# KyleHuang9/YOLO-LP

Measured on AMD Instinct MI355X. Metric: images/sec (640×640) end-to-end detect+NMS, yololps, 1/2/4/8 MI355X, higher is better.
Workload: dtype f16; 1 GPU; yololps 640x640 bs=32/GPU f16, synthetic frames resident in HBM, seeded random-init weights (sigma 0.25), conf 0.40 iou 0.45 max_det 1000; global_batch=32, parallelism=dp1: images sharded, all-gather of detections

## Files before the change

include/lp_hip.h:

```cpp
#ifndef LP_HIP_H
#define LP_HIP_H

#include <stddef.h>
#include <stdint.h>

#ifdef __cplusplus
extern "C" {
#endif

typedef enum { LP_OK = 0, LP_ERR_ARG = -1, LP_ERR_STATE = -2, LP_ERR_HIP = -3, LP_ERR_UNSUPPORTED = -4 } lp_status;
typedef enum { LP_F16 = 0, LP_BF16 = 1, LP_F32 = 2 } lp_dtype;
typedef enum { LP_ACT_NONE = 0, LP_ACT_RELU = 1, LP_ACT_SILU = 2 } lp_act;

#define LP_PRED_COLS 290
#define LP_DET_COLS 28
#define LP_MAX_SRC 4

typedef struct lp_engine lp_engine;

const char* lp_version(void);
const char* lp_last_error(void);

int lp_engine_create(lp_engine** out, int act_dtype );
void lp_engine_destroy(lp_engine* e);
// ... 201 lines not shown
    uint16_t taps[LP_REDACT_MAX_RADIUS + 1];
    uint16_t taps_c[LP_REDACT_MAX_RADIUS + 1];
} lp_redact_gauss_params;
size_t lp_redact_gauss_workspace_bytes(const lp_redact_desc* desc, int n_frames, const lp_redact_gauss_params* p);
int lp_redact_gauss_batch(const lp_redact_desc* desc, int n_frames, const float* det, const int32_t* count, int max_det,
                          const lp_redact_gauss_params* p, int32_t* status ,
                          void* workspace, size_t workspace_bytes, void* stream);

#define LP_LOOKBACK_MAX_DEPTH 32
size_t lp_lookback_state_bytes(int n_streams, int max_tracks, int depth, int rows);
int lp_lookback_update(void* state, int n_streams, int max_tracks, int depth, int max_back, int back_cap,
                       const float* det_hold, const int32_t* count_hold, const int32_t* tid, const int32_t* slot,
                       int B, int max_det, int hold_rows,
                       const int* stream_of , const unsigned char* flush ,
                       float* rel_det, int32_t* rel_count, int32_t* rel_frame,
                       float* tail_det, int32_t* tail_count, int32_t* tail_frame, void* stream);

#define LP_WATCH_MAX_ENTRIES (1 << 24)
#define LP_WATCH_MAX_COST 32768
#define LP_WATCH_BLOCK_ENTRIES 2048
#define LP_WATCH_QUERY_BLOCK 16
size_t lp_watch_workspace_bytes(int n_streams, int max_ended);
int lp_watch_match(const unsigned char* entries, int n_entries, const unsigned char* confuse ,
                   const int32_t* ended_i, const float* ended_f, const int32_t* ended_count, int n_streams, int max_ended,
                   int max_mismatch, int max_cost, int32_t* match_i, void* workspace, size_t workspace_bytes, void* stream);

#define LP_MERGE_MAX_TILES 64
#define LP_TILE_GATE_TILE_WORDS 8
typedef struct lp_tile_gate_desc {
    const unsigned char* p0;
    int pitch0;
    int h0, w0;
    int format;
    unsigned short* blocks;
} lp_tile_gate_desc;
int lp_tile_gate_luma_batch(const lp_tile_gate_desc* desc, int n_frames, void* stream);
int lp_tile_gate_update(const lp_tile_gate_desc* desc, int n_frames, const int* stream_of , int n_streams,
                        const int32_t* tiles, const int* n_tiles , int max_tiles,
                        unsigned short* ref, long long ref_elems, int32_t* age, int thres16, int min_cells, int refresh,
                        unsigned char* flag, int32_t* ncell, void* stream);

enum { LP_EVAL_TRUE = 0, LP_EVAL_PRED = 1, LP_EVAL_PRED_BINS = 2, LP_EVAL_COR = 12, LP_EVAL_CLS = 22, LP_EVAL_RIGHT = 32,
       LP_EVAL_UNBINNED = 42, LP_EVAL_NCOUNTS = 43 };
int lp_eval_counts(const float* det, const int32_t* det_count, int max_det, const float* tgt, const int32_t* tgt_count,
                   int max_t, int B, long long* counts, void* stream);

int lp_check_sigmoid_monotone(unsigned long long* dev_violations, void* stream);

int lp_check_iou_predicate(const float* dev_pairs, long long n, double iou_thres, unsigned char* dev_out, void* stream);

int lp_debug_poison_lds(void* stream);

int lp_plan_stem_tile(int fused, int Ho, int Wo, int choice, int* TH, int* TW, int* hpitch);
int lp_plan_block_tile(int variant, int Ho, int Wo, int B, int nct, int choice, int* TH, int* TW, int* hpitch);

#ifdef __cplusplus
}
#endif
#endif
```

yolo-lp_amd/csrc/lp_conv.hip:

```cpp
#include "lp_internal.h"

#include <cstdlib>

namespace lp {

int conv_launch_f16(int cfg, int mode, int ksize, int stride, int nbuf, const ConvArgs& a, hipStream_t st);
int conv_launch_bf16(int cfg, int mode, int ksize, int stride, int nbuf, const ConvArgs& a, hipStream_t st);
int conv_launch_f32(int cfg, int mode, int ksize, int stride, int nbuf, const ConvArgs& a, hipStream_t st);

int conv_stream_launch_f16(int wc, const ConvArgs& a, int cb_pack, int lds, hipStream_t st);
int conv_stream_launch_bf16(int wc, const ConvArgs& a, int cb_pack, int lds, hipStream_t st);
int conv_stream_launch_f32(int wc, const ConvArgs& a, int cb_pack, int lds, hipStream_t st);

int conv_pipe_launch_f16(int pcfg, const ConvArgs& a, int ncu, hipStream_t st);
int conv_pipe_launch_bf16(int pcfg, const ConvArgs& a, int ncu, hipStream_t st);

int head_rows_launch_f16(const ConvArgs& a, int cb_pack, hipStream_t st);
int head_rows_launch_bf16(const ConvArgs& a, int cb_pack, hipStream_t st);
int head_rows_launch_f32(const ConvArgs& a, int cb_pack, hipStream_t st);
int head_box_det_launch_f16(const ConvArgs& a, int cb_pack, hipStream_t st);
int head_box_det_launch_bf16(const ConvArgs& a, int cb_pack, hipStream_t st);
int head_box_det_launch_f32(const ConvArgs& a, int cb_pack, hipStream_t st);

ConvShape conv_shape(int dtype, int cfg, int ksize, int stride) {
// ... 226 lines not shown
    const ConvShape s = conv_pipe_shape(pcfg);
    if (pipe_is_16v(pcfg) && (nct * s.CB > 512 || nchunks > 32)) return false;
    return s.CB == cb_pack && nct * s.CB <= 1024 && nchunks <= 64;
}

static int g_ncu[16] = {0};
int device_cus() {
    int dev = 0;
    if (hipGetDevice(&dev) != hipSuccess || dev < 0 || dev >= 16) return 256;
    if (!g_ncu[dev]) {
        int n = 0;
        if (hipDeviceGetAttribute(&n, hipDeviceAttributeMultiprocessorCount, dev) != hipSuccess || n < 8) n = 256;
        g_ncu[dev] = n / 8 * 8;
        if (const char* cap = getenv("LP_PIPE_MAXWG")) { const int c = atoi(cap) / 8 * 8; if (c >= 8 && c < g_ncu[dev]) g_ncu[dev] = c; }
    }
    return g_ncu[dev];
}

bool stem_planar_tile(int Ho, int Wo, int choice, int* TH, int* TW) {
    struct Cand { long long tiles; int th, tw; };
    std::vector<Cand> cands;
    for (int tw = 4; tw <= 512 && tw < Wo + 4; tw += 4) {
        int th = 512 / tw;
        if (th > Ho) th = Ho;
        while (th >= 1 && ((th + 2) * 6 + 2) * (tw / 4 + 2) * 16 > 20 * 1024) --th;
        if (th < 1) continue;
        cands.push_back({(long long)ceil_div(Ho, th) * ceil_div(Wo, tw), th, tw});
    }
    std::sort(cands.begin(), cands.end(), [](const Cand& x, const Cand& y) { return x.tiles != y.tiles ? x.tiles < y.tiles : x.tw > y.tw; });
    if (choice < 0 || choice >= (int)cands.size()) return false;
    *TH = cands[choice].th;
    *TW = cands[choice].tw;
    return true;
}

bool stem2_fused_tile(int Ho, int Wo, int choice, int* TH, int* TW, int* hpitch) {
    struct Cand { long long cost; int th, tw; };
    std::vector<Cand> cands;
    for (int tw = 2; tw <= 128 && tw < Wo + 2; tw += 2)
        for (int th = 1; th <= 128 / tw && th <= Ho; ++th) {
            const int hp4 = tw / 2 + 2, rin = 2 * th + 3, hps = 2 * tw + 1;
            const int ntb = (th * tw + 31) / 32;
            if ((rin * 6 + 2) * hp4 * 16 > 21 * 1024 || (rin * 6 * hp4 + 63) / 64 > 24 || (2 * th + 1) * hps > 640 || ntb * 2 > 16) continue;
            cands.push_back({(long long)ceil_div(Ho, th) * ceil_div(Wo, tw) * (2 * th + 1) * hps, th, tw});
        }
    std::sort(cands.begin(), cands.end(), [](const Cand& x, const Cand& y) { return x.cost != y.cost ? x.cost < y.cost : x.tw > y.tw; });
    if (choice < 0 || choice >= (int)cands.size()) return false;
    *TH = cands[choice].th;
    *TW = cands[choice].tw;
    *hpitch = 2 * cands[choice].tw + 1;
    return true;
}

int conv_pipe_launch(int dtype, int pcfg, const ConvArgs& a, hipStream_t st) {
    if (pcfg == PIPE_P || pcfg == PIPE_FUSED2 || pcfg == PIPE_FUSED_PW || pcfg == PIPE_FUSED_BF) {
        switch (dtype) {
            case LP_F16: return conv_pipe_launch_f16(pcfg, a, device_cus(), st);
            case LP_BF16: return conv_pipe_launch_bf16(pcfg, a, device_cus(), st);
        }
        return fail(LP_ERR_UNSUPPORTED, "planar stem: 16-bit frames only");
    }
    const ConvShape s = conv_pipe_shape(pcfg);
    if (pipe_is_16s2(pcfg)) {
        const int hh2 = 2 * a.TH + 1, hw2 = 2 * a.TW + 1, nchunks = a.chunk_begin[a.nsrc];
        if (a.TH < 1 || a.TW < 1 || a.TH * a.TW > s.PB || a.hpitch != hw2 || hh2 * a.hpitch > s.HPMAX)
            return fail(LP_ERR_ARG, "conv3x3 s2p16: tile does not fit the kernel configuration");
        if (a.tiles_x * a.TW < a.Wo || a.tiles_y * a.TH < a.Ho) return fail(LP_ERR_ARG, "conv3x3 s2p16: tiles do not cover the output");
        if (a.nsrc < 1 || a.nsrc > LP_MAX_SRC || a.nct < 1 || a.nct * s.CB > 512 || nchunks < 1 || nchunks > 64 || a.nphase != 1 || a.out_scale != 1 ||
            a.H != 2 * a.Ho || a.W != 2 * a.Wo || a.out2)
            return fail(LP_ERR_ARG, "conv3x3 s2p16: not a 3x3 stride-2 layer this kernel runs");
        const int stride = a.out_pix_stride > a.res_cs ? a.out_pix_stride : a.res_cs;
        if (((long long)a.TH * a.Wo + a.TW) * stride + 2048 >= (1ll << 31)) return fail(LP_ERR_ARG, "conv3x3 s2p16: a tile's rows span more than 2^31 elements");
        switch (dtype) {
            case LP_F16: return conv_pipe_launch_f16(pcfg, a, device_cus(), st);
            case LP_BF16: return conv_pipe_launch_bf16(pcfg, a, device_cus(), st);
        }
        return fail(LP_ERR_UNSUPPORTED, "conv3x3 s2p16: 16-bit activations only");
    }
    const int hh = a.TH + 2, hw = a.TW + 2;
    if (pcfg < 0 || (pcfg >= PIPE_COUNT && !pipe_is_16(pcfg))) return fail(LP_ERR_ARG, "conv3x3 pipe: configuration");
    if (pipe_is_16(pcfg) && (a.chunk_begin[a.nsrc] < 4 || a.chunk_begin[a.nsrc] % 4 != 0)) return fail(LP_ERR_ARG, "conv3x3 pipe16: K-chunks not a multiple of four");
    if (a.TH < 1 || a.TW < 1 || a.TH * a.TW > s.PB || a.hpitch < hw || hh * a.hpitch > s.HPMAX)
        return fail(LP_ERR_ARG, "conv3x3 pipe: tile does not fit the kernel configuration");
    if (a.tiles_x * a.TW < a.Wo || a.tiles_y * a.TH < a.Ho) return fail(LP_ERR_ARG, "conv3x3 pipe: tiles do not cover the output");
    if (pipe_is_16v(pcfg) && (a.nct * s.CB > 512 || a.chunk_begin[a.nsrc] > 32)) return fail(LP_ERR_ARG, "conv3x3 pipe16v: layer exceeds the kernel's LDS tables");
    if (pipe_is_16v(pcfg)) {
        int stride = a.out_pix_stride > a.res_cs ? a.out_pix_stride : a.res_cs;
        if (a.out2 && a.out2_pix_stride > stride) stride = a.out2_pix_stride;
        if (((long long)a.TH * a.Wo + a.TW) * stride + 2048 >= (1ll << 31)) return fail(LP_ERR_ARG, "conv3x3 pipe16v: a tile's rows span more than 2^31 elements");
    }
    if (a.chunk_begin[a.nsrc] > 64) return fail(LP_ERR_ARG, "conv3x3 pipe: more K-chunks than the kernel's LDS chunk table holds");
    if (a.nsrc < 1 || a.nsrc > LP_MAX_SRC || a.nct < 1 || a.nct * s.CB > 1024 || a.nphase != 1 || a.out_scale != 1 || a.Ho != a.H || a.Wo != a.W)
        return fail(LP_ERR_ARG, "conv3x3 pipe: not a 3x3 stride-1 layer this kernel runs");
    switch (dtype) {
        case LP_F16: return conv_pipe_launch_f16(pcfg, a, device_cus(), st);
        case LP_BF16: return conv_pipe_launch_bf16(pcfg, a, device_cus(), st);
    }
    return fail(LP_ERR_UNSUPPORTED, "conv3x3 pipe: 16-bit activations only");
}

bool head_rows_fits(int dtype, int nchunks, int cb_pack, int out_c) {
    const long lds = (long)nchunks * 9 * 32 * 128 + 9 * 32 * 4 + 32 * 8 + 32 * 1168;
    return nchunks >= 1 && nchunks <= 3 && lds <= 160 * 1024 && (cb_pack == 32 || cb_pack == 64 || cb_pack == 128) && out_c == LP_PRED_COLS - 13;
}
bool head_det_fits(int dtype, int nchunks, int cb_pack, int out_c) {
    const long lds = (long)nchunks * 9 * 32 * 128 + 9 * 32 * 4 + 32 * 8 * 4 + 16 + 6 * 32 * 8 * 4 + 6 * 1168;
    return nchunks >= 1 && nchunks <= (dtype == LP_F32 ? 3 : 4) && lds <= 160 * 1024 && (cb_pack == 32 || cb_pack == 64 || cb_pack == 128) &&
           out_c == LP_PRED_COLS - 13;
}

bool head_box_det_fits(const ConvArgs& a, int cb_pack, int ksize, int stride) {
    const int nchunks = a.chunk_begin[a.nsrc];
    return ksize == 1 && stride == 1 && a.nsrc == 1 && nchunks >= 1 && nchunks <= 4 && a.reg_bins == 1 && a.out_c == 12 && a.nct == 1 &&
           cb_pack >= 32 && a.nphase == 1 && a.out_scale == 1 && a.Ho == a.H && a.Wo == a.W && a.src[0].cs % 8 == 0;
}
int head_box_det_launch(int dtype, const ConvArgs& a, int cb_pack, hipStream_t st) {
    if (!a.det_mode || !a.out || !a.zero || !head_box_det_fits(a, cb_pack, 1, 1)) return fail(LP_ERR_ARG, "head box: op does not fit");
    if (a.out_pix_stride % 4 != 0 || a.out_img_stride % 4 != 0 || ((uintptr_t)a.out & 15)) return fail(LP_ERR_ARG, "head box: candidate rows are not 16-byte aligned");
    switch (dtype) {
        case LP_F16: return head_box_det_launch_f16(a, cb_pack, st);
        case LP_BF16: return head_box_det_launch_bf16(a, cb_pack, st);
        case LP_F32: return head_box_det_launch_f32(a, cb_pack, st);
    }
    return fail(LP_ERR_ARG, "head box: dtype");
}

int head_rows_launch(int dtype, const ConvArgs& a, int cb_pack, hipStream_t st) {
    const int nchunks = a.chunk_begin[a.nsrc];
    if (!(a.det_mode ? head_det_fits(dtype, nchunks, cb_pack, a.out_c) : head_rows_fits(dtype, nchunks, cb_pack, a.out_c)))
        return fail(LP_ERR_ARG, "head rows: op does not fit");
    const int kc = 128 / (int)dtype_size(dtype);
    for (int i = 0; i < a.nsrc; ++i)
        if (a.src[i].cs % (kc / 4) != 0)
            return fail(LP_ERR_ARG, "head rows: source channels are not whole 32-byte K-steps");
    if (a.nphase != 1 || a.out_scale != 1 || a.Ho != a.H || a.Wo != a.W || !a.out) return fail(LP_ERR_ARG, "head rows: bad geometry");
    switch (dtype) {
        case LP_F16: return head_rows_launch_f16(a, cb_pack, st);
        case LP_BF16: return head_rows_launch_bf16(a, cb_pack, st);
        case LP_F32: return head_rows_launch_f32(a, cb_pack, st);
    }
    return fail(LP_ERR_ARG, "head rows: dtype");
}

}

extern "C" int lp_plan_block_tile(int variant, int Ho, int Wo, int B, int nct, int choice, int* TH, int* TW, int* hpitch) {
    const int pcfg = variant - LP_VARIANT_PIPE_D;
    if (!TH || !TW || Ho < 1 || Wo < 1 || B < 1 || nct < 1) return lp::fail(LP_ERR_ARG, "lp_plan_block_tile: bad arguments");
    if (!lp::pipe_is_16v(pcfg) && !lp::pipe_is_16s2(pcfg)) return lp::fail(LP_ERR_UNSUPPORTED, "lp_plan_block_tile: not a block-tiled variant");
    const lp::ConvShape s = lp::conv_pipe_shape(pcfg);
    const int stride = lp::pipe_is_16s2(pcfg) ? 2 : 1;
    lp::conv_pick_tile16v(s, Ho, Wo, B, nct, choice, TH, TW, stride);
    if (hpitch) *hpitch = (*TW - 1) * stride + 3;
    return LP_OK;
}

extern "C" int lp_plan_stem_tile(int fused, int Ho, int Wo, int choice, int* TH, int* TW, int* hpitch) {
    if (!TH || !TW || Ho < 1 || Wo < 1) return lp::fail(LP_ERR_ARG, "lp_plan_stem_tile: bad arguments");
    int hp = 0;
    const bool ok = fused ? lp::stem2_fused_tile(Ho, Wo, choice, TH, TW, &hp) : lp::stem_planar_tile(Ho, Wo, choice, TH, TW);
    if (hpitch) *hpitch = hp;
    return ok ? LP_OK : LP_ERR_UNSUPPORTED;
}
```

yolo-lp_amd/csrc/lp_engine.hip:

```cpp
#include "lp_internal.h"

#include <cmath>
#include <cstdlib>
#include <cstring>
#include <map>
#include <utility>
#include <vector>

namespace lp {

static thread_local std::string g_err;
void set_error(const std::string& msg) { g_err = msg; }
int fail(int code, const std::string& msg) {
    g_err = msg;
    return code;
}

enum OpKind { OP_INPUT = 0, OP_CONV = 1, OP_DECONV = 2, OP_POOL = 3, OP_HEAD_CLS = 4, OP_HEAD_BOX = 5 };

struct Tensor {
    int c, cs, sl;
    bool unused = false;
    size_t offset;
    int h, w;
// ... 761 lines not shown
    L.cb_pack = cb_pack;
    if (op.planar) {
        Launch& P = e->stem_planar;
        P = L;
        ConvArgs& pa = P.a;
        if (pa.W % 4 != 0 || !stem_planar_tile(pa.Ho, pa.Wo, op.planar - 1, &pa.TH, &pa.TW))
            return fail(LP_ERR_UNSUPPORTED, "planar stem: no tile for this frame size");
        pa.tw_magic = (unsigned)(((1u << 22) + pa.TW - 1) / pa.TW);
        pa.tiles_x = ceil_div(pa.Wo, pa.TW);
        pa.tiles_y = ceil_div(pa.Ho, pa.TH);
        pa.src[0].ptr = nullptr;
        P.pipe = PIPE_P + 1;
    }
    if (op.fused) {
        const Op& stem = e->ops[1];
        Launch& F = e->stem2_fused;
        F = L;
        ConvArgs& fa = F.a;
        if (!stem2_fused_tile(fa.Ho, fa.Wo, op.fused - 1, &fa.TH, &fa.TW, &fa.hpitch))
            return fail(LP_ERR_UNSUPPORTED, "fused stem: no tile for this frame size");
        fa.tw_magic = (unsigned)(((1u << 22) + fa.TW - 1) / fa.TW);
        fa.hp_magic = (unsigned)(((1u << 22) + fa.hpitch - 1) / fa.hpitch);
        fa.tiles_x = ceil_div(fa.Wo, fa.TW);
        fa.tiles_y = ceil_div(fa.Ho, fa.TH);
        fa.src[0].ptr = nullptr;
        fa.fz_w1 = e->dev_w + stem.w_off;
        fa.fz_b1 = (const float*)(e->dev_w + stem.b_off);
        fa.fz_act1 = stem.act;
        fa.fz_c1 = e->tensors[stem.dst].cs;
        F.pipe = PIPE_FUSED2 + 1;
    }
    if (op.fused_bf) {
        const Op& up = e->ops[op.bf_up];
        const Op& c1 = e->ops[op.bf_cv1];
        Launch& F = e->bf_fused[(int)idx];
        F = L;
        ConvArgs& fa = F.a;
        fa.src[0].ptr = tptr(up.src[0]); fa.src[0].cs = e->tensors[up.src[0]].cs;
        fa.src[1].ptr = tptr(c1.src[0]); fa.src[1].cs = e->tensors[c1.src[0]].cs;
        fa.fz_w1 = e->dev_w + c1.w_off;
        fa.fz_b1 = (const float*)(e->dev_w + c1.b_off);
        fa.fz_act1 = c1.act;
        fa.bf_wd = e->dev_w + up.w_off;
        fa.bf_bd = (const float*)(e->dev_w + up.b_off);
        fa.bf_wd_phase_stride = up.w_phase_stride;
        F.pipe = PIPE_FUSED_BF + 1;
    }
    if (op.fused_pw) {
        const Op& pw = e->ops[idx - 1];
        Launch& F = e->pw_fused[(int)idx];
        F = L;
        ConvArgs& fa = F.a;
        int hp = 0;
        if (!stem2_fused_tile(fa.Ho, fa.Wo, op.fused_pw - 1, &fa.TH, &fa.TW, &hp))
            return fail(LP_ERR_UNSUPPORTED, "fused 1x1 + 3x3 s2: no tile for this map size");
        fa.hpitch = hp;
        fa.tw_magic = (unsigned)(((1u << 22) + fa.TW - 1) / fa.TW);
        fa.hp_magic = (unsigned)(((1u << 22) + fa.hpitch - 1) / fa.hpitch);
        fa.tiles_x = ceil_div(fa.Wo, fa.TW);
        fa.tiles_y = ceil_div(fa.Ho, fa.TH);
        fa.src[0].ptr = tptr(pw.src[0]);
        fa.src[0].cs = e->tensors[pw.src[0]].cs;
        fa.fz_w1 = e->dev_w + pw.w_off;
        fa.fz_b1 = (const float*)(e->dev_w + pw.b_off);
        fa.fz_act1 = pw.act;
        fa.fz_c1 = e->tensors[pw.dst].cs;
        F.pipe = PIPE_FUSED_PW + 1;
    }
    return LP_OK;
}

static bool stem_planar_possible(const lp_engine* e) {
    return e->dtype != LP_F32 && e->ops.size() > 1 && e->ops[0].kind == OP_INPUT && e->ops[0].s2d && e->ops[1].kind == OP_CONV &&
           e->ops[1].ksize == 3 && e->ops[1].stride == 1 && e->ops[1].mode == MODE_ACT && e->ops[1].nct == 1 && e->ops[1].nchunks == 1 &&
           (conv_shape(e->dtype, e->ops[1].cfg, 3, 1).CB == 32 || conv_shape(e->dtype, e->ops[1].cfg, 3, 1).CB == 64) && e->ops[1].res < 0 &&
           e->ops[1].dst2 < 0;
}
static bool frame_direct(const lp_engine* e, const void* x, int x_dtype) { return x_dtype == e->dtype && ((uintptr_t)x & 15) == 0; }
static bool stem_planar_now(const lp_engine* e, const void* x, int x_dtype) { return e->ops.size() > 1 && e->ops[1].planar && frame_direct(e, x, x_dtype); }
static bool stem2_fused_possible(const lp_engine* e) {
    if (!stem_planar_possible(e) || e->ops.size() < 3) return false;
    const Op& s = e->ops[1];
    const Op& c = e->ops[2];
    if (c.kind != OP_CONV || c.ksize != 3 || c.stride != 2 || c.nsrc != 1 || c.src[0] != s.dst || c.res >= 0 || c.dst2 >= 0 || c.mode != MODE_ACT ||
        c.nct != 1 || c.nphase != 1 || c.nchunks < 1 || c.nchunks > 2 || s.act != LP_ACT_RELU || c.act != LP_ACT_RELU) return false;
    const int cb = conv_shape(e->dtype, c.cfg, 3, 2).CB, cs2 = e->tensors[c.dst].cs;
    if ((cb != 32 && cb != 64) || cb != 32 * ((cs2 + 31) / 32) || e->tensors[s.dst].cs > 16 * c.nchunks) return false;
    for (size_t i = 3; i < e->ops.size(); ++i) {
        const Op& o = e->ops[i];
        for (int k = 0; k < o.nsrc; ++k) if (o.src[k] == s.dst) return false;
        if (o.res == s.dst) return false;
    }
    return true;
}
static bool pw_fused_possible(const lp_engine* e, size_t i) {
    if (e->dtype == LP_F32 || i < 2 || i >= e->ops.size()) return false;
    const Op& p = e->ops[i - 1];
    const Op& c = e->ops[i];
    if (c.kind != OP_CONV || c.ksize != 3 || c.stride != 2 || c.nsrc != 1 || c.res >= 0 || c.dst2 >= 0 || c.mode != MODE_ACT || c.nct != 1 || c.nphase != 1) return false;
    if (p.kind != OP_CONV || p.ksize != 1 || p.stride != 1 || p.nsrc != 1 || p.res >= 0 || p.dst2 >= 0 || p.mode != MODE_ACT || p.nct != 1 || p.nphase != 1 ||
        p.nchunks != 1 || p.dst != c.src[0] || p.lane != c.lane || p.signal) return false;
    const int cs0 = e->tensors[p.src[0]].cs, cs1 = e->tensors[p.dst].cs, cs2 = e->tensors[c.dst].cs;
    if (cs0 != 64 || (cs1 != 32 && cs1 != 64) || (cs2 != 32 && cs2 != 64)) return false;
    if (conv_shape(e->dtype, p.cfg, 1, 1).CB != cs1 || conv_shape(e->dtype, c.cfg, 3, 2).CB != cs2 || c.nchunks != cs1 / 16) return false;
    for (size_t k = 0; k < e->ops.size(); ++k) {
        if (k == i) continue;
        const Op& o = e->ops[k];
// ... 775 lines not shown
```

yolo-lp_amd/csrc/lp_internal.h:

```cpp
#pragma once
#include <hip/hip_runtime.h>
#include <stdint.h>
#include <stddef.h>
#include <atomic>
#include <string>

#include "../../include/lp_hip.h"

#ifndef LP_PRO_ORDER
#define LP_PRO_ORDER 0
#endif

namespace lp {

typedef _Float16 f16;
typedef __bf16 bf16;

void set_error(const std::string& msg);
int fail(int code, const std::string& msg);
#define LP_HIP_CHECK(expr)                                                                       \
    do {                                                                                         \
        hipError_t _e = (expr);                                                                  \
        if (_e != hipSuccess)                                                                    \
            return ::lp::fail(LP_ERR_HIP, std::string(#expr) + ": " + hipGetErrorString(_e));    \
// ... 62 lines not shown
    const void* zero;
    void* trash;
    void* out;
    void* out2;
    int out_split;
    int out2_pix_stride;
    long long out2_img_stride;
    const void* res;
    int res_cs;
    float alpha;
    int B, H, W;
    int Ho, Wo;
    int TH, TW, tiles_x, tiles_y;
    unsigned tw_magic, hp_magic;
    int hpitch;
    int nct;
    int out_c;
    long long out_img_stride;
    int out_pix_stride;
    int out_scale;
    int nphase;
    long long w_phase_stride;
    int act;
    int det_mode;
    unsigned long long* det_keys;
    int* det_cnt;
    int det_np, det_n, det_anchor0;
    float det_conf;
    const int* det_prev;
    int* det_snap;
    const void* fz_w1;
    const float* fz_b1;
    int fz_act1, fz_c1;
    const void* bf_wd;
    const float* bf_bd;
    long long bf_wd_phase_stride;
    int reg_bins;
    const float* proj;
    float stride_px;
};

struct ConvShape {
    int CB, PB, KC, HPMAX, NT, WP, WGC, WGP;
};
ConvShape conv_shape(int dtype, int cfg, int ksize, int stride);
void conv_pick_tile(const ConvShape& s, int ksize, int stride, int Ho, int Wo, int choice, int* TH, int* TW);
int conv_pick_pitch(const ConvShape& s, int dtype, int ksize, int stride, int TH, int TW);
int conv_pick_pitch16(const ConvShape& s, int TH, int TW);
void conv_pick_tile16v(const ConvShape& s, int Ho, int Wo, int B, int nct, int choice, int* TH, int* TW, int stride = 1);
int device_cus();
int conv_launch(int dtype, int cfg, int mode, int ksize, int stride, int nbuf, const ConvArgs& a, hipStream_t st);
bool stem_planar_tile(int Ho, int Wo, int choice, int* TH, int* TW);
bool stem2_fused_tile(int Ho, int Wo, int choice, int* TH, int* TW, int* hpitch);

int conv_stream_lds(int dtype, int wc, int nchunks, int cb_pack);
int conv_stream_launch(int dtype, int wc, const ConvArgs& a, int cb_pack, hipStream_t st);

ConvShape conv_pipe_shape(int pcfg);
bool conv_pipe_fits(int dtype, int pcfg, int cb_pack, int ksize, int stride, int mode, int nct, int nphase, int nchunks);
int conv_pipe_launch(int dtype, int pcfg, const ConvArgs& a, hipStream_t st);

bool head_rows_fits(int dtype, int nchunks, int cb_pack, int out_c);
bool head_det_fits(int dtype, int nchunks, int cb_pack, int out_c);
bool head_box_det_fits(const ConvArgs& a, int cb_pack, int ksize, int stride);
int head_box_det_launch(int dtype, const ConvArgs& a, int cb_pack, hipStream_t st);
int head_rows_launch(int dtype, const ConvArgs& a, int cb_pack, hipStream_t st);

struct NmsWs {
    int32_t* cnt;
    unsigned long long* keys;
    float* rows;
    float4* sbox;
    int32_t* kept;
    int NP;
    size_t bytes;
};
NmsWs nms_carve(void* base, int B, int N);
int nms_score_launch(float* pred, int B, int rows_per_img, int anchor0, int N, float conf_f, const NmsWs& w, bool write_box, hipStream_t st);
int zero_counts_launch(int* p, int n, hipStream_t st);

int input_launch(const void* x, int x_dtype, void* dst, int dtype, int B, int H, int W, hipStream_t st);
int input_s2d_launch(const void* x, int x_dtype, void* dst, int dtype, int B, int H, int W, hipStream_t st);
size_t pool_min_lds_bytes(int dtype, int h, int w);
constexpr size_t POOL_MAX_LDS = 128 * 1024;
int pool_launch(const void* src, void* d1, void* d2, void* d3, int dtype, int B, int h, int w, int cs, hipStream_t st);

}
```

yolo-lp_amd/csrc/lp_pw_s2_fused.inc:

```
#pragma once
#include "lp_conv_kernel.inc"
#include <type_traits>

namespace lp {

constexpr int PW_MAXPOS = 640;
constexpr int PW_PX = 128;

template <typename T, int NCB1, int NCB2>
__global__ __launch_bounds__(512, 2) void pw_s2_fused_kernel(const ConvArgs a, const int total) {
    typedef typename Mma<T>::V V;
    static_assert(sizeof(T) == 2, "16-bit activations only");
    constexpr int NW = 8, NCH2 = 2 * NCB1, CB1 = 32 * NCB1, CB2 = 32 * NCB2;
    constexpr int STB = PW_MAXPOS * 32;
    constexpr int W2B = NCH2 * 9 * CB2 * 32;
    __shared__ __attribute__((aligned(1024))) char stile[NCH2 * STB], w2l[W2B];
    __shared__ __attribute__((aligned(16))) float bias1_lds[64], bias2_lds[64];

    const int tid = threadIdx.x, lane = tid & 63, wave = __builtin_amdgcn_readfirstlane(tid >> 6);
    const int r = lane & 31, h = lane >> 5;
    const int G = gridDim.x;
    const int TH = a.TH, TW = a.TW;
    const int HS = a.H, WS = a.W;
    const int HWE = TW + 1, HPS = a.hpitch;
    const int SH = 2 * TH + 1, SW = 2 * TW + 1;
    const int npos = SH * HPS;
    const int tpi = a.tiles_y * a.tiles_x;
    const int cs0 = a.src[0].cs;
    const T* const x = (const T*)a.src[0].ptr;

    V fa1[NCB1][4];
    {
        const char* wp = (const char*)a.fz_w1 + r * 128;
#pragma unroll
        for (int cb = 0; cb < NCB1; ++cb)
#pragma unroll
            for (int kb = 0; kb < 4; ++kb) fa1[cb][kb] = *(const V*)(wp + cb * 32 * 128 + swz(r, 2 * kb + h, 8) * 16);
#pragma unroll
        for (int cb = 0; cb < NCB1; ++cb)
#pragma unroll
            for (int kb = 0; kb < 4; ++kb) asm volatile("" ::"v"(fa1[cb][kb]));
    }
    if (tid < 64) bias1_lds[tid] = tid < CB1 ? a.fz_b1[tid] : 0.f;
    if (tid < 64) bias2_lds[tid] = tid < CB2 ? a.bias[tid] : 0.f;
    for (int i = tid; i < W2B / 16; i += 512) ((uint4*)w2l)[i] = ((const uint4*)a.w)[i];
    __syncthreads();

    const int nsegA = (npos + 31) / 32;
    const int npix = TH * TW;
    const int nsegB = (npix + 31) / 32;
    const int ntB = nsegB * NCB2;
    constexpr int MAXA = (PW_MAXPOS / 32 + NW - 1) / NW;
    constexpr int MAXB = (PW_PX / 32 * NCB2 + NW - 1) / NW;
    T* const trash = (T*)a.trash;

    for (int t = blockIdx.x; t < total; t += G) {
        const int b = t / tpi, trem = t - b * tpi;
        const int ty0 = (trem / a.tiles_x) * TH, tx0 = (trem % a.tiles_x) * TW;
        const T* const xb = x + (long long)b * HS * WS * cs0;

        V fb[MAXA][4];
        bool live[MAXA];
#pragma unroll
        for (int kA = 0; kA < MAXA; ++kA) {
            const int p = (wave + kA * NW) * 32 + r;
            const int sy = (int)(((unsigned)p * a.hp_magic) >> 22), cp = p - sy * HPS;
            const int sx = cp < HWE ? 2 * cp : 2 * (cp - HWE) + 1;
            const int Y = 2 * ty0 - 1 + sy, X = 2 * tx0 - 1 + sx;
            live[kA] = p < npos && cp < SW && Y >= 0 && Y < HS && X >= 0 && X < WS;
            const T* const px = xb + ((long long)Y * WS + X) * cs0 + 8 * h;
#pragma unroll
            for (int kb = 0; kb < 4; ++kb) {
                V v = {};
                if (live[kA]) v = *(const V*)(px + 16 * kb);
                fb[kA][kb] = v;
            }
        }
        __syncthreads();
#pragma unroll
        for (int kA = 0; kA < MAXA; ++kA) {
            if (wave + kA * NW >= nsegA) break;
            const int p = (wave + kA * NW) * 32 + r;
#pragma unroll
            for (int cb = 0; cb < NCB1; ++cb) {
                f32x16 acc;
#pragma unroll
                for (int rg = 0; rg < 4; ++rg) {
                    const f32x4 bv = *(const f32x4*)(bias1_lds + cb * 32 + 4 * h + 8 * rg);
#pragma unroll
                    for (int e = 0; e < 4; ++e) acc[4 * rg + e] = bv[e];
                }
#pragma unroll
                for (int kb = 0; kb < 4; ++kb) acc = Mma<T>::mma(fa1[cb][kb], fb[kA][kb], acc);
                act_dispatch(a.fz_act1, [&](auto tag) {
                    constexpr int ACT = decltype(tag)::value;
#pragma unroll
                    for (int pr = 0; pr < 2; ++pr) {
                        typedef T T4 __attribute__((ext_vector_type(4)));
                        union { T4 v; unsigned u[2]; } qa, qb;
#pragma unroll
                        for (int k = 0; k < 4; ++k) {
                            qa.v[k] = from_f32<T>(act_c<ACT>(acc[8 * pr + k]));
                            qb.v[k] = from_f32<T>(act_c<ACT>(acc[8 * pr + 4 + k]));
                        }
                        const auto s0 = __builtin_amdgcn_permlane32_swap(qa.u[0], qb.u[0], false, false);
                        const auto s1 = __builtin_amdgcn_permlane32_swap(qa.u[1], qb.u[1], false, false);
                        uint4 v = {s0[0], s1[0], s0[1], s1[1]};
                        const bool keep = live[kA] && cb * 32 + 16 * pr + 8 * h < a.fz_c1;
                        if (!keep) v = uint4{0u, 0u, 0u, 0u};
                        if (p < PW_MAXPOS) *(uint4*)(stile + (cb * 2 + pr) * STB + p * 32 + swz(p, h, 2) * 16) = v;
                    }
                });
            }
        }
        __syncthreads();

        T* const out = (T*)a.out + (long long)b * a.out_img_stride;
#pragma unroll
        for (int kB = 0; kB < MAXB; ++kB) {
            const int iB = wave + kB * NW;
            if (iB >= ntB) break;
            const int cb = iB % NCB2, sg = iB / NCB2;
            int pl = sg * 32 + r;
            const bool inpix = pl < npix;
            if (!inpix) pl = 0;
            const int ty = (int)(((unsigned)pl * a.tw_magic) >> 22), tx = pl - ty * TW;
            f32x16 acc;
#pragma unroll
            for (int rg = 0; rg < 4; ++rg) {
                const f32x4 bv = *(const f32x4*)(bias2_lds + cb * 32 + 4 * h + 8 * rg);
#pragma unroll
                for (int e = 0; e < 4; ++e) acc[4 * rg + e] = bv[e];
            }
            const char* const wl = w2l + (cb * 32 + r) * 32 + swz(r, h, 2) * 16;
            int boff[9];
#pragma unroll
            for (int tp = 0; tp < 9; ++tp) {
                const int ky = tp / 3, kx = tp - ky * 3;
                const int sx = 2 * tx + kx;
                const int pos = (2 * ty + ky) * HPS + ((sx & 1) ? HWE + (sx >> 1) : (sx >> 1));
                boff[tp] = pos * 32 + swz(pos, h, 2) * 16;
            }
            const unsigned sb_ = (unsigned)(size_t)(const __attribute__((address_space(3))) char*)stile;
            const unsigned wb_ = (unsigned)(size_t)(const __attribute__((address_space(3))) char*)wl;
#pragma unroll
            for (int q = 0; q < NCH2; ++q) {
                V fbq[9], fw[9];
                asm volatile("s_waitcnt lgkmcnt(0)" ::: "memory");
#pragma unroll
                for (int tp = 0; tp < 9; ++tp) {
                    const unsigned ab = sb_ + q * STB + boff[tp], aw = wb_ + (q * 9 + tp) * CB2 * 32;
                    asm volatile("ds_read_b128 %0, %1" : "=v"(fbq[tp]) : "v"(ab));
                    asm volatile("ds_read_b128 %0, %1" : "=v"(fw[tp]) : "v"(aw));
                }
#pragma unroll
                for (int tp = 0; tp < 9; ++tp) {
                    const int left = 16 - 2 * tp;
                    if (left >= 15) asm volatile("s_waitcnt lgkmcnt(15)" : "+v"(fbq[tp]), "+v"(fw[tp])::"memory");
                    else if (left == 14) asm volatile("s_waitcnt lgkmcnt(14)" : "+v"(fbq[tp]), "+v"(fw[tp])::"memory");
                    else if (left == 12) asm volatile("s_waitcnt lgkmcnt(12)" : "+v"(fbq[tp]), "+v"(fw[tp])::"memory");
                    else if (left == 10) asm volatile("s_waitcnt lgkmcnt(10)" : "+v"(fbq[tp]), "+v"(fw[tp])::"memory");
                    else if (left == 8) asm volatile("s_waitcnt lgkmcnt(8)" : "+v"(fbq[tp]), "+v"(fw[tp])::"memory");
                    else if (left == 6) asm volatile("s_waitcnt lgkmcnt(6)" : "+v"(fbq[tp]), "+v"(fw[tp])::"memory");
                    else if (left == 4) asm volatile("s_waitcnt lgkmcnt(4)" : "+v"(fbq[tp]), "+v"(fw[tp])::"memory");
                    else if (left == 2) asm volatile("s_waitcnt lgkmcnt(2)" : "+v"(fbq[tp]), "+v"(fw[tp])::"memory");
                    else asm volatile("s_waitcnt lgkmcnt(0)" : "+v"(fbq[tp]), "+v"(fw[tp])::"memory");
                    acc = Mma<T>::mma(fw[tp], fbq[tp], acc);
                }
            }
            const int oy = ty0 + ty, ox = tx0 + tx;
            const bool pok = inpix && oy < a.Ho && ox < a.Wo;
            const long long opix = (long long)oy * a.Wo + ox;
            act_dispatch(a.act, [&](auto tag) {
                constexpr int ACT = decltype(tag)::value;
#pragma unroll
                for (int pr = 0; pr < 2; ++pr) {
                    typedef T T4 __attribute__((ext_vector_type(4)));
                    union { T4 v; unsigned u[2]; } qa, qb;
#pragma unroll
                    for (int k = 0; k < 4; ++k) {
                        qa.v[k] = from_f32<T>(act_c<ACT>(acc[8 * pr + k]));
                        qb.v[k] = from_f32<T>(act_c<ACT>(acc[8 * pr + 4 + k]));
                    }
                    const auto s0 = __builtin_amdgcn_permlane32_swap(qa.u[0], qb.u[0], false, false);
                    const auto s1 = __builtin_amdgcn_permlane32_swap(qa.u[1], qb.u[1], false, false);
                    const uint4 v = {s0[0], s1[0], s0[1], s1[1]};
                    const int c = cb * 32 + 8 * h + 16 * pr;
                    if (pok && c < a.out_c) *(uint4*)(out + opix * a.out_pix_stride + c) = v;
                }
            });
        }
        (void)trash;
    }
}

template <typename T>
static inline int pw_s2_fused_launch(const ConvArgs& a, int ncu, hipStream_t st) {
    const int ncb1 = (a.fz_c1 + 31) / 32, ncb2 = (a.out_c + 31) / 32;
    if (a.TH < 1 || a.TW < 1 || a.TH * a.TW > PW_PX || a.hpitch < 2 * a.TW + 1 || (2 * a.TH + 1) * a.hpitch > PW_MAXPOS)
        return fail(LP_ERR_ARG, "fused 1x1 + 3x3 s2: tile does not fit");
    if (a.nsrc != 1 || a.nct != 1 || a.chunk_begin[1] != 2 * ncb1 || ncb1 < 1 || ncb1 > 2 || ncb2 < 1 || ncb2 > 2 || a.res || a.src[0].cs < 64 ||
        a.src[0].cs % 8 != 0 || !a.fz_w1 || !a.fz_b1 || a.fz_c1 % 16 != 0 || a.out_c % 8 != 0 || ((uintptr_t)a.w & 15) != 0)
        return fail(LP_ERR_ARG, "fused 1x1 + 3x3 s2: not a pair this kernel runs");
    const int total = a.B * a.tiles_y * a.tiles_x;
    const int grid = total < ncu ? total : ncu;
    auto launch = [&](auto kernel) {
        hipLaunchKernelGGL(kernel, dim3((unsigned)grid), dim3(512), 0, st, a, total);
        hipError_t e = hipGetLastError();
        if (e != hipSuccess) return fail(LP_ERR_HIP, std::string("fused 1x1 + 3x3 s2 launch: ") + hipGetErrorString(e));
        return (int)LP_OK;
    };
    if (ncb1 == 2 && ncb2 == 2) return launch(pw_s2_fused_kernel<T, 2, 2>);
    if (ncb1 == 1 && ncb2 == 1) return launch(pw_s2_fused_kernel<T, 1, 1>);
    if (ncb1 == 2 && ncb2 == 1) return launch(pw_s2_fused_kernel<T, 2, 1>);
    return launch(pw_s2_fused_kernel<T, 1, 2>);
}

}
```

yolo-lp_amd/yolov6/hip/abi.py:

```python
import ctypes
import os
from ctypes import POINTER, c_char_p, c_double, c_float, c_int, c_int32, c_size_t, c_void_p

LP_F16, LP_BF16, LP_F32 = 0, 1, 2
LP_ACT_NONE, LP_ACT_RELU, LP_ACT_SILU = 0, 1, 2
LP_PRED_COLS, LP_DET_COLS, LP_MAX_SRC = 290, 28, 4
LP_VARIANT_STREAM64, LP_VARIANT_STREAM128, LP_VARIANT_ROWS = 16, 17, 18
LP_VARIANT_PIPE_D, LP_VARIANT_PIPE_B, LP_VARIANT_PIPE_F, LP_VARIANT_PIPE_C = 32, 33, 34, 35
LP_VARIANT_PIPE16_D, LP_VARIANT_PIPE16_F = 39, 41
LP_VARIANT_PIPE16_V0, LP_VARIANT_PIPE16_V1 = 42, 43
LP_VARIANT_PIPE16_S2A, LP_VARIANT_PIPE16_S2B = 48, 49
LP_VARIANT_FUSED_BIFUSION = 45
LP_VARIANT_BOX_SPARSE, LP_VARIANT_BOX_DENSE = 46, 47
LP_VARIANT_FUSED_PW_S2 = 38
LP_VARIANT_FUSED_STEM2 = 37
LP_VARIANT_PIPE_P = 36
VARIANT_SHORT = {
    LP_VARIANT_STREAM64: 'S', LP_VARIANT_STREAM128: 'W', LP_VARIANT_ROWS: 'R',
    LP_VARIANT_PIPE_D: 'Pd', LP_VARIANT_PIPE_B: 'Pb', LP_VARIANT_PIPE_F: 'Pf', LP_VARIANT_PIPE_C: 'Pc', LP_VARIANT_PIPE_P: 'Pp',
    LP_VARIANT_FUSED_STEM2: 'Fz', LP_VARIANT_FUSED_PW_S2: 'Fp', LP_VARIANT_FUSED_BIFUSION: 'Fb',
    LP_VARIANT_PIPE16_D: 'Md', LP_VARIANT_PIPE16_F: 'Mf', LP_VARIANT_PIPE16_V0: 'V0', LP_VARIANT_PIPE16_V1: 'V1',
    LP_VARIANT_PIPE16_S2A: 'Xa', LP_VARIANT_PIPE16_S2B: 'Xb',
}
LP_FRAMES_PER_LAUNCH = 64
# ... 114 lines not shown
    'lp_engine_set_op_variant': (c_int, [c_void_p, c_int, c_int, c_int]),
    'lp_engine_set_op_tile': (c_int, [c_void_p, c_int, c_int]),
    'lp_engine_op_tile': (c_int, [c_void_p, c_int, POINTER(c_int), POINTER(c_int), POINTER(c_int)]),
    'lp_engine_copy_tuning': (c_int, [c_void_p, c_void_p]),
    'lp_nms_workspace_bytes': (c_size_t, [c_int, c_int]),
    'lp_nms_candidate_counts': (c_void_p, [c_void_p, c_int, c_int]),
    'lp_preprocess_letterbox': (c_int, [c_void_p, c_int, c_int, c_void_p, c_int, c_int, c_int, c_int, c_int, c_int, c_int,
                                        c_void_p]),
    'lp_rescale_round': (c_int, [c_void_p, c_int, c_double, c_double, c_double, c_int, c_int, c_void_p]),
    'lp_preprocess_letterbox_batch': (c_int, [POINTER(FrameDesc), c_int, c_int, c_void_p, c_int, c_int, c_int, c_void_p]),
    'lp_rescale_round_batch': (c_int, [c_void_p, c_void_p, c_int, c_int, POINTER(RescaleDesc), c_void_p]),
    'lp_preprocess_tiles_batch': (c_int, [POINTER(TileDesc), c_int, c_int, c_void_p, c_int, c_int, c_int, c_void_p]),
    'lp_preprocess_nv12_batch': (c_int, [POINTER(Nv12Desc), c_int, c_int, c_void_p, c_int, c_int, c_int, c_void_p]),
    'lp_nv12_to_bgr_batch': (c_int, [POINTER(Nv12BgrDesc), c_int, c_void_p]),
    'lp_merge_tiles_workspace_bytes': (c_size_t, [c_int, c_int]),
    'lp_merge_tiles': (c_int, [c_void_p, c_void_p, POINTER(TileRef), c_int, c_int, POINTER(c_int), c_int, c_double, c_int, c_int, c_int,
                               c_void_p, c_void_p, c_void_p, c_void_p, c_size_t, c_void_p]),
    'lp_track_state_bytes': (c_size_t, [c_int, c_int]),
    'lp_track_dropped_offset': (c_size_t, [c_int, c_int]),
    'lp_track_update': (c_int, [c_void_p, c_int, c_int, POINTER(TrackParams), c_void_p, c_void_p, c_int, c_int, POINTER(c_int),
                                c_void_p, c_void_p, c_void_p, c_void_p, c_void_p, c_void_p, c_int, c_void_p]),
    'lp_track_update_slots': (c_int, [c_void_p, c_int, c_int, POINTER(TrackParams), c_void_p, c_void_p, c_int, c_int, POINTER(c_int),
                                      c_void_p, c_void_p, c_void_p, c_void_p, c_void_p, c_void_p, c_void_p, c_int, c_void_p]),
    'lp_track_update_hold': (c_int, [c_void_p, c_int, c_int, POINTER(TrackParams), c_void_p, c_void_p, c_int, c_int, POINTER(c_int),
                                     c_void_p, c_void_p, c_void_p, c_void_p, c_void_p, c_void_p, c_void_p, c_int,
                                     POINTER(TrackHoldParams), c_void_p, c_void_p, c_void_p, c_void_p]),
    'lp_plate_crops_batch': (c_int, [POINTER(CropDesc), c_int, c_void_p, c_void_p, c_int, c_void_p, c_void_p, c_int, c_int, c_int,
                                     c_void_p]),
    'lp_crop_sharpness': (c_int, [c_void_p, c_void_p, c_int, c_int, c_int, c_void_p, c_void_p]),
    'lp_best_shot_state_bytes': (c_size_t, [c_int, c_int, c_int, c_int]),
    'lp_best_shot_update': (c_int, [c_void_p, c_int, c_int, c_int, c_int, c_void_p, c_void_p, c_int, c_int, c_void_p, c_void_p, c_void_p,
                                    c_void_p, c_void_p, c_int, POINTER(c_int), c_void_p, c_void_p, c_int, c_double, c_void_p, c_void_p,
                                    c_void_p, c_void_p, c_void_p]),
    'lp_redact_workspace_bytes': (c_size_t, [POINTER(RedactDesc), c_int, POINTER(RedactParams)]),
    'lp_redact_plates_batch': (c_int, [POINTER(RedactDesc), c_int, c_void_p, c_void_p, c_int, POINTER(RedactParams), c_void_p, c_void_p,
                                       c_size_t, c_void_p]),
    'lp_redact_gauss_workspace_bytes': (c_size_t, [POINTER(RedactDesc), c_int, POINTER(RedactGaussParams)]),
    'lp_redact_gauss_batch': (c_int, [POINTER(RedactDesc), c_int, c_void_p, c_void_p, c_int, POINTER(RedactGaussParams), c_void_p, c_void_p,
                                      c_size_t, c_void_p]),
    'lp_lookback_state_bytes': (c_size_t, [c_int, c_int, c_int, c_int]),
    'lp_lookback_update': (c_int, [c_void_p, c_int, c_int, c_int, c_int, c_int, c_void_p, c_void_p, c_void_p, c_void_p, c_int, c_int, c_int,
                                   POINTER(c_int), c_void_p, c_void_p, c_void_p, c_void_p, c_void_p, c_void_p, c_void_p, c_void_p]),
    'lp_watch_workspace_bytes': (c_size_t, [c_int, c_int]),
    'lp_watch_match': (c_int, [c_void_p, c_int, c_void_p, c_void_p, c_void_p, c_void_p, c_int, c_int, c_int, c_int, c_void_p, c_void_p,
                               c_size_t, c_void_p]),
    'lp_tile_gate_luma_batch': (c_int, [POINTER(TileGateDesc), c_int, c_void_p]),
    'lp_tile_gate_update': (c_int, [POINTER(TileGateDesc), c_int, POINTER(c_int), c_int, c_void_p, POINTER(c_int), c_int, c_void_p,
                                    ctypes.c_longlong, c_void_p, c_int, c_int, c_int, c_void_p, c_void_p, c_void_p]),
    'lp_eval_counts': (c_int, [c_void_p, c_void_p, c_int, c_void_p, c_void_p, c_int, c_int, c_void_p, c_void_p]),
    'lp_check_sigmoid_monotone': (c_int, [c_void_p, c_void_p]),
    'lp_debug_poison_lds': (c_int, [c_void_p]),
    'lp_check_iou_predicate': (c_int, [c_void_p, ctypes.c_longlong, c_double, c_void_p, c_void_p]),
    'lp_plan_stem_tile': (c_int, [c_int, c_int, c_int, c_int, c_void_p, c_void_p, c_void_p]),
    'lp_plan_block_tile': (c_int, [c_int, c_int, c_int, c_int, c_int, c_int, c_void_p, c_void_p, c_void_p]),
    'lp_nms': (c_int, [c_void_p, c_int, c_int, c_double, c_double, c_int, c_void_p, c_void_p, c_void_p, c_void_p,
                       c_size_t, c_void_p]),
}

_lib = None


def load():
    global _lib
    if _lib is None:
        import torch
        if not os.path.exists(LIB_PATH):
            raise RuntimeError('HIP extension %s is missing: build it with `make -C %s` (or '
                               '`python -c "import __graft_entry__ as g; g.build()"`). The GPU path has no '
                               'eager fallback.' % (LIB_PATH, CSRC_DIR))
        lib = ctypes.CDLL(LIB_PATH)
        for name, (restype, argtypes) in SYMBOLS.items():
            fn = getattr(lib, name)
            fn.restype = restype
            fn.argtypes = argtypes
        _lib = lib
    return _lib


def check(rc, what=''):
    if rc < 0:
        msg = load().lp_last_error()
        raise RuntimeError('%s failed (%d): %s' % (what or 'libyololp_hip', rc, msg.decode() if msg else '?'))
    return rc
```

Baseline: 17620 images/s.

## Warp-specialize fused 1x1+3x3 s2 kernel with double-buffered LDS tiles

Splits the fused pointwise + stride-2 3x3 kernel into producer waves, which load input and compute the 1x1 stage into LDS, and consumer waves, which run the 3x3 stage. The two groups alternate over a double-buffered intermediate tile, so stage A of the next tile overlaps stage B of the current one, and the per-tile pair of __syncthreads becomes a single barrier. To fit two buffers in LDS, the tile size is halved (max positions 640→320, pixels 128→64), a dedicated tile planner is added, and the two-blocks-per-CU launch bound is dropped. It also adds a debug cap on the fused grid size. In exchange, each stage now gets only half the waves, occupancy is lower, and tiles are smaller with more halo overhead.

```diff
diff --git a/include/lp_hip.h b/include/lp_hip.h
--- a/include/lp_hip.h
+++ b/include/lp_hip.h
@@ -277,6 +277,8 @@
 int lp_debug_poison_lds(void* stream);
 
 int lp_plan_stem_tile(int fused, int Ho, int Wo, int choice, int* TH, int* TW, int* hpitch);
+int lp_plan_pw_s2_tile(int Ho, int Wo, int choice, int* TH, int* TW, int* hpitch);
+int lp_debug_set_fused_grid_cap(int n);
 int lp_plan_block_tile(int variant, int Ho, int Wo, int B, int nct, int choice, int* TH, int* TW, int* hpitch);
 
 #ifdef __cplusplus
diff --git a/yolo-lp_amd/csrc/lp_conv.hip b/yolo-lp_amd/csrc/lp_conv.hip
--- a/yolo-lp_amd/csrc/lp_conv.hip
+++ b/yolo-lp_amd/csrc/lp_conv.hip
@@ -302,11 +302,32 @@
     return true;
 }
 
+bool pw_s2_fused_tile(int Ho, int Wo, int choice, int* TH, int* TW, int* hpitch) {
+    struct Cand { long long cost; int th, tw; };
+    std::vector<Cand> cands;
+    for (int tw = 1; tw <= 64 && tw <= Wo; ++tw)
+        for (int th = 1; th <= 64 / tw && th <= Ho; ++th) {
+            const int pos = (2 * th + 1) * (2 * tw + 1);
+            if (pos > 320) continue;
+            cands.push_back({(long long)ceil_div(Ho, th) * ceil_div(Wo, tw) * pos, th, tw});
+        }
+    std::sort(cands.begin(), cands.end(), [](const Cand& x, const Cand& y) { return x.cost != y.cost ? x.cost < y.cost : x.tw > y.tw; });
+    if (choice < 0 || choice >= (int)cands.size()) return false;
+    *TH = cands[choice].th;
+    *TW = cands[choice].tw;
+    *hpitch = 2 * cands[choice].tw + 1;
+    return true;
+}
+
+static int g_fused_wg_cap = 0;
+
 int conv_pipe_launch(int dtype, int pcfg, const ConvArgs& a, hipStream_t st) {
     if (pcfg == PIPE_P || pcfg == PIPE_FUSED2 || pcfg == PIPE_FUSED_PW || pcfg == PIPE_FUSED_BF) {
+        int ncu = device_cus();
+        if ((pcfg == PIPE_FUSED2 || pcfg == PIPE_FUSED_PW) && g_fused_wg_cap > 0 && g_fused_wg_cap < ncu) ncu = g_fused_wg_cap;
         switch (dtype) {
-            case LP_F16: return conv_pipe_launch_f16(pcfg, a, device_cus(), st);
-            case LP_BF16: return conv_pipe_launch_bf16(pcfg, a, device_cus(), st);
+            case LP_F16: return conv_pipe_launch_f16(pcfg, a, ncu, st);
+            case LP_BF16: return conv_pipe_launch_bf16(pcfg, a, ncu, st);
         }
         return fail(LP_ERR_UNSUPPORTED, "planar stem: 16-bit frames only");
     }
@@ -405,6 +426,20 @@
     return LP_OK;
 }
 
+extern "C" int lp_plan_pw_s2_tile(int Ho, int Wo, int choice, int* TH, int* TW, int* hpitch) {
+    if (!TH || !TW || Ho < 1 || Wo < 1) return lp::fail(LP_ERR_ARG, "lp_plan_pw_s2_tile: bad arguments");
+    int hp = 0;
+    const bool ok = lp::pw_s2_fused_tile(Ho, Wo, choice, TH, TW, &hp);
+    if (hpitch) *hpitch = hp;
+    return ok ? LP_OK : LP_ERR_UNSUPPORTED;
+}
+
+extern "C" int lp_debug_set_fused_grid_cap(int n) {
+    if (n < 0) return lp::fail(LP_ERR_ARG, "lp_debug_set_fused_grid_cap: negative cap");
+    lp::g_fused_wg_cap = n;
+    return LP_OK;
+}
+
 extern "C" int lp_plan_stem_tile(int fused, int Ho, int Wo, int choice, int* TH, int* TW, int* hpitch) {
     if (!TH || !TW || Ho < 1 || Wo < 1) return lp::fail(LP_ERR_ARG, "lp_plan_stem_tile: bad arguments");
     int hp = 0;
diff --git a/yolo-lp_amd/csrc/lp_engine.hip b/yolo-lp_amd/csrc/lp_engine.hip
--- a/yolo-lp_amd/csrc/lp_engine.hip
+++ b/yolo-lp_amd/csrc/lp_engine.hip
@@ -837,7 +837,7 @@
         F = L;
         ConvArgs& fa = F.a;
         int hp = 0;
-        if (!stem2_fused_tile(fa.Ho, fa.Wo, op.fused_pw - 1, &fa.TH, &fa.TW, &hp))
+        if (!pw_s2_fused_tile(fa.Ho, fa.Wo, op.fused_pw - 1, &fa.TH, &fa.TW, &hp))
             return fail(LP_ERR_UNSUPPORTED, "fused 1x1 + 3x3 s2: no tile for this map size");
         fa.hpitch = hp;
         fa.tw_magic = (unsigned)(((1u << 22) + fa.TW - 1) / fa.TW);
diff --git a/yolo-lp_amd/csrc/lp_internal.h b/yolo-lp_amd/csrc/lp_internal.h
--- a/yolo-lp_amd/csrc/lp_internal.h
+++ b/yolo-lp_amd/csrc/lp_internal.h
@@ -138,6 +138,7 @@
 int conv_launch(int dtype, int cfg, int mode, int ksize, int stride, int nbuf, const ConvArgs& a, hipStream_t st);
 bool stem_planar_tile(int Ho, int Wo, int choice, int* TH, int* TW);
 bool stem2_fused_tile(int Ho, int Wo, int choice, int* TH, int* TW, int* hpitch);
+bool pw_s2_fused_tile(int Ho, int Wo, int choice, int* TH, int* TW, int* hpitch);
 
 int conv_stream_lds(int dtype, int wc, int nchunks, int cb_pack);
 int conv_stream_launch(int dtype, int wc, const ConvArgs& a, int cb_pack, hipStream_t st);
diff --git a/yolo-lp_amd/csrc/lp_pw_s2_fused.inc b/yolo-lp_amd/csrc/lp_pw_s2_fused.inc
--- a/yolo-lp_amd/csrc/lp_pw_s2_fused.inc
+++ b/yolo-lp_amd/csrc/lp_pw_s2_fused.inc
@@ -4,17 +4,20 @@
 
 namespace lp {
 
-constexpr int PW_MAXPOS = 640;
-constexpr int PW_PX = 128;
+constexpr int PW_MAXPOS = 320;
+constexpr int PW_PX = 64;
+constexpr int PW_NWA = 4, PW_NWB = 4;
 
 template <typename T, int NCB1, int NCB2>
-__global__ __launch_bounds__(512, 2) void pw_s2_fused_kernel(const ConvArgs a, const int total) {
+__global__ __launch_bounds__(512) void pw_s2_fused_kernel(const ConvArgs a, const int total) {
     typedef typename Mma<T>::V V;
     static_assert(sizeof(T) == 2, "16-bit activations only");
-    constexpr int NW = 8, NCH2 = 2 * NCB1, CB1 = 32 * NCB1, CB2 = 32 * NCB2;
+    constexpr int NWA = PW_NWA, NWB = PW_NWB, NCH2 = 2 * NCB1, CB1 = 32 * NCB1, CB2 = 32 * NCB2;
     constexpr int STB = PW_MAXPOS * 32;
+    constexpr int TILEB = NCH2 * STB;
     constexpr int W2B = NCH2 * 9 * CB2 * 32;
-    __shared__ __attribute__((aligned(1024))) char stile[NCH2 * STB], w2l[W2B];
+    static_assert(2 * TILEB + W2B + 512 <= 160 * 1024, "two intermediate tiles + the resident weights + the biases: one CU's LDS");
+    __shared__ __attribute__((aligned(1024))) char stile[2 * TILEB], w2l[W2B];
     __shared__ __attribute__((aligned(16))) float bias1_lds[64], bias2_lds[64];
 
     const int tid = threadIdx.x, lane = tid & 63, wave = __builtin_amdgcn_readfirstlane(tid >> 6);
@@ -28,9 +31,15 @@
     const int tpi = a.tiles_y * a.tiles_x;
     const int cs0 = a.src[0].cs;
     const T* const x = (const T*)a.src[0].ptr;
+    const bool producer = wave < NWA;
+    const int wa = wave, wb = wave - NWA;
 
     V fa1[NCB1][4];
-    {
+#pragma unroll
+    for (int cb = 0; cb < NCB1; ++cb)
+#pragma unroll
+        for (int kb = 0; kb < 4; ++kb) fa1[cb][kb] = V{};
+    if (producer) {
         const char* wp = (const char*)a.fz_w1 + r * 128;
 #pragma unroll
         for (int cb = 0; cb < NCB1; ++cb)
@@ -50,24 +59,28 @@
     const int npix = TH * TW;
     const int nsegB = (npix + 31) / 32;
     const int ntB = nsegB * NCB2;
-    constexpr int MAXA = (PW_MAXPOS / 32 + NW - 1) / NW;
-    constexpr int MAXB = (PW_PX / 32 * NCB2 + NW - 1) / NW;
-    T* const trash = (T*)a.trash;
-
-    for (int t = blockIdx.x; t < total; t += G) {
+    constexpr int MAXA = (PW_MAXPOS / 32 + NWA - 1) / NWA;
+    constexpr int MAXB = (PW_PX / 32 * NCB2 + NWB - 1) / NWB;
+
+    V fb[MAXA][4];
+    bool live[MAXA];
+#pragma unroll
+    for (int kA = 0; kA < MAXA; ++kA) {
+        live[kA] = false;
+#pragma unroll
+        for (int kb = 0; kb < 4; ++kb) fb[kA][kb] = V{};
+    }
+    auto request = [&](int kA, int t) __attribute__((always_inline)) {
+        const bool any = t < total;
         const int b = t / tpi, trem = t - b * tpi;
         const int ty0 = (trem / a.tiles_x) * TH, tx0 = (trem % a.tiles_x) * TW;
         const T* const xb = x + (long long)b * HS * WS * cs0;
-
-        V fb[MAXA][4];
-        bool live[MAXA];
-#pragma unroll
-        for (int kA = 0; kA < MAXA; ++kA) {
-            const int p = (wave + kA * NW) * 32 + r;
+        {
+            const int p = (wa + kA * NWA) * 32 + r;
             const int sy = (int)(((unsigned)p * a.hp_magic) >> 22), cp = p - sy * HPS;
             const int sx = cp < HWE ? 2 * cp : 2 * (cp - HWE) + 1;
             const int Y = 2 * ty0 - 1 + sy, X = 2 * tx0 - 1 + sx;
-            live[kA] = p < npos && cp < SW && Y >= 0 && Y < HS && X >= 0 && X < WS;
+            live[kA] = any && p < npos && cp < SW && Y >= 0 && Y < HS && X >= 0 && X < WS;
             const T* const px = xb + ((long long)Y * WS + X) * cs0 + 8 * h;
 #pragma unroll
             for (int kb = 0; kb < 4; ++kb) {
@@ -76,11 +89,11 @@
                 fb[kA][kb] = v;
             }
         }
-        __syncthreads();
-#pragma unroll
-        for (int kA = 0; kA < MAXA; ++kA) {
-            if (wave + kA * NW >= nsegA) break;
-            const int p = (wave + kA * NW) * 32 + r;
+    };
+    auto stage_a = [&](int kA, int buf) __attribute__((always_inline)) {
+        char* const st = stile + buf * TILEB;
+        if (wa + kA * NWA < nsegA) {
+            const int p = (wa + kA * NWA) * 32 + r;
 #pragma unroll
             for (int cb = 0; cb < NCB1; ++cb) {
                 f32x16 acc;
@@ -108,17 +121,19 @@
                         uint4 v = {s0[0], s1[0], s0[1], s1[1]};
                         const bool keep = live[kA] && cb * 32 + 16 * pr + 8 * h < a.fz_c1;
                         if (!keep) v = uint4{0u, 0u, 0u, 0u};
-                        if (p < PW_MAXPOS) *(uint4*)(stile + (cb * 2 + pr) * STB + p * 32 + swz(p, h, 2) * 16) = v;
+                        if (p < PW_MAXPOS) *(uint4*)(st + (cb * 2 + pr) * STB + p * 32 + swz(p, h, 2) * 16) = v;
                     }
                 });
             }
         }
-        __syncthreads();
-
+    };
+    auto stage_b = [&](int t, int buf) __attribute__((always_inline)) {
+        const int b = t / tpi, trem = t - b * tpi;
+        const int ty0 = (trem / a.tiles_x) * TH, tx0 = (trem % a.tiles_x) * TW;
         T* const out = (T*)a.out + (long long)b * a.out_img_stride;
 #pragma unroll
         for (int kB = 0; kB < MAXB; ++kB) {
-            const int iB = wave + kB * NW;
+            const int iB = wb + kB * NWB;
             if (iB >= ntB) break;
             const int cb = iB % NCB2, sg = iB / NCB2;
             int pl = sg * 32 + r;
@@ -141,7 +156,7 @@
                 const int pos = (2 * ty + ky) * HPS + ((sx & 1) ? HWE + (sx >> 1) : (sx >> 1));
                 boff[tp] = pos * 32 + swz(pos, h, 2) * 16;
             }
-            const unsigned sb_ = (unsigned)(size_t)(const __attribute__((address_space(3))) char*)stile;
+            const unsigned sb_ = (unsigned)(size_t)(const __attribute__((address_space(3))) char*)(stile + buf * TILEB);
             const unsigned wb_ = (unsigned)(size_t)(const __attribute__((address_space(3))) char*)wl;
 #pragma unroll
             for (int q = 0; q < NCH2; ++q) {
@@ -190,7 +205,35 @@
                 }
             });
         }
-        (void)trash;
+    };
+    auto tile_barrier = [&]() __attribute__((always_inline)) {
+        asm volatile("s_waitcnt lgkmcnt(0)" ::: "memory");
+        __builtin_amdgcn_s_barrier();
+        asm volatile("" ::: "memory");
+    };
+
+    int t = blockIdx.x;
+    if (t >= total) return;
+    auto produce = [&](int buf, int tn) __attribute__((always_inline)) {
+#pragma unroll
+        for (int kA = 0; kA < MAXA; ++kA) {
+            stage_a(kA, buf);
+            request(kA, tn);
+        }
+    };
+    if (producer) {
+#pragma unroll
+        for (int kA = 0; kA < MAXA; ++kA) request(kA, t);
+        produce(0, t + G);
+    }
+    tile_barrier();
+    for (int cur = 0; t < total; t += G, cur ^= 1) {
+        if (producer) {
+            if (t + G < total) produce(cur ^ 1, t + 2 * G);
+        } else {
+            stage_b(t, cur);
+        }
+        tile_barrier();
     }
 }
 
diff --git a/yolo-lp_amd/yolov6/hip/abi.py b/yolo-lp_amd/yolov6/hip/abi.py
--- a/yolo-lp_amd/yolov6/hip/abi.py
+++ b/yolo-lp_amd/yolov6/hip/abi.py
@@ -190,6 +190,8 @@
     'lp_debug_poison_lds': (c_int, [c_void_p]),
     'lp_check_iou_predicate': (c_int, [c_void_p, ctypes.c_longlong, c_double, c_void_p, c_void_p]),
     'lp_plan_stem_tile': (c_int, [c_int, c_int, c_int, c_int, c_void_p, c_void_p, c_void_p]),
+    'lp_plan_pw_s2_tile': (c_int, [c_int, c_int, c_int, c_void_p, c_void_p, c_void_p]),
+    'lp_debug_set_fused_grid_cap': (c_int, [c_int]),
     'lp_plan_block_tile': (c_int, [c_int, c_int, c_int, c_int, c_int, c_int, c_void_p, c_void_p, c_void_p]),
     'lp_nms': (c_int, [c_void_p, c_int, c_int, c_double, c_double, c_int, c_void_p, c_void_p, c_void_p, c_void_p,
                        c_size_t, c_void_p]),
```

Result: no change. 17560 images/s (-0.4%).
